# frank-xwang/InstanceDiffusion

Measured on AMD Instinct MI355X. Metric: images/sec at 512x512, 50 PLMS steps, N=8 instances (Multi-instance Sampler), higher is better.
Workload: dtype bf16; 1 GPU; C3: SD-1.5 InstanceDiffusion UNet (1.228B params, seeded random weights), 64x64 latent (512x512), 50 PLMS steps, CFG 7.5, N=8 boxes, MIS 0.36, alpha [0.8,0,0.2]; images_per_gpu=32, unet_forwards_per_image=406

## Files before the change

include/idf.h:

```cpp
#ifndef IDF_H_
#define IDF_H_

#include <stdint.h>

#ifdef __cplusplus
extern "C" {
#endif

#define IDF_ABI_VERSION 5

enum { IDF_BF16 = 0, IDF_F16 = 1 };
enum { IDF_E_ARG = -1, IDF_E_ALIGN = -2, IDF_E_UNSUPPORTED = -3 };

enum {
  IDF_EPI_BIAS     = 1,
  IDF_EPI_ROWBIAS  = 2,
  IDF_EPI_RES      = 4,
  IDF_EPI_GATE     = 8,
  IDF_EPI_SILU     = 16,
  IDF_EPI_GELU     = 32,
  IDF_EPI_GEGLU    = 64,
  IDF_EPI_OUT_F32  = 128,
  IDF_EPI_OUT_NCHW = 256,
  IDF_EPI_LN_ROW   = 512,
// ... 49 lines not shown

typedef struct {
  const void* x; const void* W; void* out;
  const float* bias; const void* rowbias; const void* res;
  int B, Hin, Win, Cin, Cout;
  int stride;
  int upsample;
  int ldx, ldo, ldr, ld_rowbias;
  int n_valid;
  int epi; int dtype;
  void* ws; long long ws_bytes;
  float* gn_partial;
} idf_conv3x3_args;
int idf_conv3x3(const idf_conv3x3_args* a, void* stream);
int idf_conv3x3_down(const idf_conv3x3_args* a, void* stream);

int idf_conv_in(const float* x_nchw, const float* w , const float* bias, void* out,
                int B, int Cin, int H, int W, int Cout, int dtype, void* stream);

typedef struct {
  const void* q; int ldq; long long strideQ; int nq;
  const void* k0; int ldk0; long long strideK0; const void* vt0; int ldv0; long long strideV0; int n0;
  const void* k1; int ldk1; long long strideK1; const void* vt1; int ldv1; long long strideV1; int n1;
  void* out; int ldo; long long strideO;
  int B, H, d;
  float scale;
  int dtype;
  const void* qbits; long long strideQb;
  const void* kbits0; long long strideKb0;
  const void* kbits1; long long strideKb1;
// ... 54 lines not shown
```

instancediffusion_amd/_lib.py:

```python
from __future__ import annotations

import ctypes as C
import os

_HERE = os.path.dirname(os.path.abspath(__file__))
LIB_PATH = os.environ.get("IDF_LIB_PATH", os.path.join(_HERE, "libidf_gfx950.so"))

IDF_BF16, IDF_F16 = 0, 1
IDF_STAT_GEMM_BIG_LAUNCHES, IDF_STAT_ATTN2_LAUNCHES, IDF_STAT_GEMM_RING_LAUNCHES, IDF_STAT_ATTN8_LAUNCHES, IDF_STAT_GN_EPI_LAUNCHES = 0, 1, 2, 3, 4
IDF_STAT_QKV_ROW_LAUNCHES, IDF_STAT_GEGLU_ROW_LAUNCHES = 6, 7
IDF_TUNE_GEMM_BIG, IDF_TUNE_ATTN2, IDF_TUNE_GEMM_RING, IDF_TUNE_BIG_MIN_EFF, IDF_TUNE_ATTN8, IDF_TUNE_MLP, IDF_TUNE_QKV_ROW, IDF_TUNE_GEGLU_ROW = 0, 1, 2, 3, 4, 5, 6, 7
EPI_LN_ROW, EPI_LN_COL, EPI_GEGLU_P32 = 512, 1024, 2048
EPI_BIAS, EPI_ROWBIAS, EPI_RES, EPI_GATE, EPI_SILU, EPI_GELU, EPI_GEGLU, EPI_OUT_F32, EPI_OUT_NCHW = \
    1, 2, 4, 8, 16, 32, 64, 128, 256

vp, ll, ci, cf = C.c_void_p, C.c_longlong, C.c_int, C.c_float


class GemmArgs(C.Structure):
    _fields_ = [("A", vp), ("W", vp), ("out", vp), ("bias", vp), ("rowbias", vp), ("res", vp), ("gate", vp),
                ("M", ci), ("N", ci), ("K", ci),
                ("lda", ci), ("ldw", ci), ("ldo", ci), ("ldr", ci), ("ld_rowbias", ci),
                ("rows_per_batch", ci),
                ("batch", ci), ("strideA", ll), ("strideW", ll), ("strideO", ll), ("strideR", ll),
                ("epi", ci), ("dtype", ci), ("ws", vp), ("ws_bytes", ll),
                ("ln_stats", vp), ("stride_ln_stats", ll), ("ln_c", vp), ("ln_d", vp),
                ("out_stats", vp), ("out_stats_eps", cf),
                ("ln_eps", cf), ("ln_stats_out", vp),
                ("vt_out", vp), ("ld_vt", ci), ("vt_col0", ci)]


class ConvArgs(C.Structure):
    _fields_ = [("x", vp), ("W", vp), ("out", vp), ("bias", vp), ("rowbias", vp), ("res", vp),
                ("B", ci), ("Hin", ci), ("Win", ci), ("Cin", ci), ("Cout", ci),
                ("stride", ci), ("upsample", ci),
                ("ldx", ci), ("ldo", ci), ("ldr", ci), ("ld_rowbias", ci),
                ("n_valid", ci), ("epi", ci), ("dtype", ci), ("ws", vp), ("ws_bytes", ll), ("gn_partial", vp)]


class AttnArgs(C.Structure):
    _fields_ = [("q", vp), ("ldq", ci), ("strideQ", ll), ("nq", ci),
                ("k0", vp), ("ldk0", ci), ("strideK0", ll), ("vt0", vp), ("ldv0", ci), ("strideV0", ll), ("n0", ci),
                ("k1", vp), ("ldk1", ci), ("strideK1", ll), ("vt1", vp), ("ldv1", ci), ("strideV1", ll), ("n1", ci),
                ("out", vp), ("ldo", ci), ("strideO", ll),
                ("B", ci), ("H", ci), ("d", ci), ("scale", cf), ("dtype", ci),
                ("qbits", vp), ("strideQb", ll), ("kbits0", vp), ("strideKb0", ll), ("kbits1", vp), ("strideKb1", ll)]


class MlpArgs(C.Structure):
    _fields_ = [("x", vp), ("ldx", ci), ("ln_stats", vp), ("w1", vp), ("ldw1", ci), ("cd", vp), ("w2p", vp), ("ldw2", ci),
                ("b2", vp), ("gate", vp), ("out", vp), ("ldo", ci), ("M", ci), ("C", ci), ("dtype", ci)]


SYMBOLS = {
    "idf_abi_version": (ci, []),
    "idf_build_info": (C.c_char_p, []),
    "idf_set_tuning": (ci, [ci, ci]),
    "idf_get_stat": (ll, [ci]),
    "idf_gemm": (ci, [C.POINTER(GemmArgs), vp]),
    "idf_conv3x3": (ci, [C.POINTER(ConvArgs), vp]),
    "idf_conv3x3_down": (ci, [C.POINTER(ConvArgs), vp]),
    "idf_mlp_geglu": (ci, [C.POINTER(MlpArgs), vp]),
    "idf_conv_in": (ci, [vp, vp, vp, vp, ci, ci, ci, ci, ci, ci, vp]),
    "idf_attention": (ci, [C.POINTER(AttnArgs), vp]),
    "idf_groupnorm_ws_floats": (ll, [ci, ci]),
    "idf_groupnorm": (ci, [vp, vp, vp, vp, vp, ci, ci, ci, cf, ci, ci, vp]),
    "idf_groupnorm_stats": (ci, [vp, vp, ci, ci, ci, ci, ci, vp]),
    "idf_groupnorm_apply": (ci, [vp, vp, vp, vp, vp, ci, ci, ci, ci, cf, ci, ci, vp]),
    "idf_layernorm": (ci, [vp, ci, vp, ci, vp, vp, ci, ci, cf, ci, vp]),
    "idf_row_stats": (ci, [vp, ci, vp, ci, ci, cf, ci, vp]),
    "idf_layernorm_patch2": (ci, [vp, vp, ci, vp, vp, ci, ci, ci, ci, cf, ci, vp]),
    "idf_seg_in_conv": (ci, [vp, vp, vp, vp, ci, ci, ci, ci, ci, vp]),
    "idf_dwconv7x7": (ci, [vp, vp, vp, vp, ci, ci, ci, ci, ci, vp]),
    "idf_scaleu_concat": (ci, [vp, vp, vp, vp, vp, vp, ci, ci, ci, ci, ci, ci, vp]),
    "idf_timestep_embedding": (ci, [vp, vp, ci, ci, ci, vp]),
    "idf_unifusion_embed": (ci, [vp, vp, vp, vp, vp, vp, vp, vp, ci, ci, ci, ci, vp]),
# ... 43 lines not shown
```

instancediffusion_amd/csrc/gemm_big.hip:

```cpp
#include "gemm_core.h"
#include <cstdlib>

using namespace idfcore;

namespace {

__device__ __attribute__((aligned(128))) unsigned short idf_zero_page[64];

#ifndef IDF_WAVE_ROWS
#define IDF_WAVE_ROWS 64
#endif
constexpr int WM = IDF_WAVE_ROWS, TM = WM / 32;
constexpr int NWAVES = 2 * 256 / WM;

template <int I> struct IC { static constexpr int value = I; };
template <int I, int N, int STEP, class F> __device__ __forceinline__ void static_for(F&& f) {
  if constexpr (I < N) { f(IC<I>{}); static_for<I + STEP, N, STEP>(f); }
}

typedef const __attribute__((address_space(1))) void* gptr_t;
typedef __attribute__((address_space(3))) void* lptr_t;

__device__ __forceinline__ unsigned lds_addr(const void* p) { return (unsigned)(size_t)p; }
__device__ __forceinline__ void dma16_sv(const void* sbase , unsigned voff_bytes, unsigned lds) {
// ... 425 lines not shown
#pragma unroll
          for (int j = 0; j < 4; ++j) {
            const f32x4 t = st4[j];
            v[2 * j] = t[1] * fmaf(-t[0], cn, v[2 * j]);
            v[2 * j + 1] = t[3] * fmaf(-t[2], cn, v[2 * j + 1]);
          }
        }
#pragma unroll
        for (int j = 0; j < 8; ++j) v[j] += bn;
        if (mb < p.M) *reinterpret_cast<u32x4*>(orow + mb) = pack8<DT>(v);
      }
    }
  });
}

#ifdef IDF_BIG_TRACE
__device__ unsigned long long idf_big_trace_buf[4][8];
#define TR_DECL unsigned long long tr_last = __builtin_readcyclecounter(), tr_acc[8] = {0, 0, 0, 0, 0, 0, 0, 0};
#define TR(i) { const unsigned long long tr_now = __builtin_readcyclecounter(); tr_acc[i] += tr_now - tr_last; tr_last = tr_now; }
#define TR_COUNT(i) { tr_acc[i] += 1; }
#define TR_DUMP { const int trb = blockIdx.x == 0 ? 0 : ((int)blockIdx.x == (int)gridDim.x / 2 ? 1 : -1);                     \
    if (trb >= 0 && lane == 0 && (wave == 0 || wave == NWAVES / 2)) { for (int i = 0; i < 8; ++i) idf_big_trace_buf[trb * 2 + (wave ? 1 : 0)][i] = tr_acc[i]; } }
#else
#define TR_DECL
#define TR(i)
#define TR_COUNT(i)
#define TR_DUMP
#endif

template <int DT, int BM, int BN, int BKT, int NSTG, bool CONV, bool SPLIT, bool LNS = false, bool VT = false, bool STATS = false,
          bool GLU = false, bool GST = false>
__global__ __launch_bounds__(64 * NWAVES, 1) void gemm_kernel_big(const CoreParams p, const int tiles_total) {
  constexpr int WN = BN / 2, TN = WN / 32;
  constexpr int NW = NWAVES;
  constexpr int RS = BKT;
  constexpr int CPR = BKT / 8;
  constexpr int RPI = 64 / CPR;
  constexpr int W_INST = BN / (RPI * NW), A_INST = BM / (RPI * NW);
  constexpr int DPW = W_INST + A_INST;
  constexpr int STAGE = (BM + BN) * RS;
  static_assert(BN % (RPI * NW) == 0 && BM % (RPI * NW) == 0, "tile rows must split evenly over the DMA instructions");
  extern __shared__ __attribute__((aligned(16))) unsigned short smem[];

  const int tid = threadIdx.x;
  const int lane = tid & 63, wave = __builtin_amdgcn_readfirstlane(tid >> 6);
  const int l31 = lane & 31, hi = lane >> 5;
// ... 13 lines not shown
  const int full = SPLIT ? p.full_items : tiles_total;
  auto item_map = [&](int item, int& tile, int& slice, int& nki) {
    if (!SPLIT || item < full) { tile = item; slice = 0; nki = SPLIT ? p.kt_full : nk; }
    else { const int r = item - full; const int t = r / S; tile = full + t; slice = r - t * S; nki = nk; }
  };

  const int dr = lane / CPR, dc = lane % CPR;
  auto swz = [](int row) { return CPR == 8 ? ((row >> 1) & 7) : ((row >> 2) & 3); };
  unsigned woff[W_INST], aoff[A_INST];
  int ayx[A_INST];
  int l_seq, l_kt = 0, l_k0 = 0, l_nk = 0, tap = 0, ci0 = 0;

  auto setup_loader = [&](int item) {
    int tile, slice;
    item_map(item, tile, slice, l_nk);
    const int m_tile = tile / tiles_n;
    const int n0 = (tile - m_tile * tiles_n) * BN, m0 = m_tile * BM;
    l_k0 = slice * nk;
#pragma unroll
    for (int j = 0; j < W_INST; ++j) {
      const int row = RPI * (wave + NW * j) + dr;
      woff[j] = (unsigned)(n0 + row) * (unsigned)p.ldw + (unsigned)((dc ^ swz(row)) * 8);
    }
#pragma unroll
    for (int j = 0; j < A_INST; ++j) {
      const int row = RPI * (wave + NW * j) + dr;
      const int m = min(m0 + row, p.M - 1);
      const unsigned sw = (unsigned)((dc ^ swz(row)) * 8);
      if (CONV) {
        const int hw = p.Ho * p.Wo;
        const int b = m / hw, rem = m - b * hw;
        const int yo = rem / p.Wo, xo = rem - yo * p.Wo;
        const int y0 = yo * p.stride - p.pad_lo, x0 = xo * p.stride - p.pad_lo;
        if (p.up == 0) {
          int mask = 0;
#pragma unroll
          for (int t = 0; t < 9; ++t) {
            const int yi = y0 + t / 3, xi = x0 + t % 3;
            mask |= ((yi >= 0) & (yi < p.Hin) & (xi >= 0) & (xi < p.Win)) << t;
          }
          ayx[j] = mask;
          aoff[j] = (unsigned)b * (unsigned)(p.Hin * p.Win) * (unsigned)p.lda + (unsigned)((y0 * p.Win + x0) * p.lda) + sw;
        } else {
          ayx[j] = (y0 << 16) | (x0 & 0xffff);
          aoff[j] = (unsigned)b * (unsigned)(p.Hin * p.Win) * (unsigned)p.lda + sw;
        }
      } else {
// ... 1 lines not shown
        aoff[j] = (unsigned)m * (unsigned)p.lda + sw;
      }
    }
    if (CONV) { const int k_elem = l_k0 * BKT; tap = k_elem / p.Cin; ci0 = k_elem - tap * p.Cin; }
  };

  auto issue_piece = [&](int stage, auto II) {
    constexpr int i = decltype(II)::value;
    unsigned short* Al = smem + stage * STAGE;
    if constexpr (i < W_INST) {
      constexpr int j = i;
      dma16_sv(p.W + (size_t)(l_k0 + l_kt) * BKT, woff[j] * 2u, lds_addr(Al + BM * RS + RPI * (wave + NW * j) * RS));
    } else {
      constexpr int j = i - W_INST;
      const unsigned dst = lds_addr(Al + RPI * (wave + NW * j) * RS);
      if (CONV && p.up == 0) {
        const int ky = tap / 3, kx = tap - ky * 3;
        const unsigned tapoff = (unsigned)((ky * p.Win + kx) * p.lda + ci0);
        const bool ok = (ayx[j] >> tap) & 1;
        const unsigned short* src = ok ? p.A + (aoff[j] + tapoff) : idf_zero_page + dc * 8;
        dma16_v(src, dst);
      } else if (CONV) {
        const int ky = tap / 3, kx = tap - ky * 3;
        const int Hup = p.Hin << p.up, Wup = p.Win << p.up;
        const int yi = (ayx[j] >> 16) + ky, xi = (int)(short)(ayx[j] & 0xffff) + kx;
        const bool ok = (yi >= 0) & (yi < Hup) & (xi >= 0) & (xi < Wup);
        const int ys = yi >> p.up, xs = xi >> p.up;
        const unsigned short* src = ok ? p.A + ci0 + (aoff[j] + (unsigned)(ys * p.Win + xs) * (unsigned)p.lda) : idf_zero_page + dc * 8;
        dma16_v(src, dst);
      } else {
        dma16_sv(p.A + (size_t)(l_k0 + l_kt) * BKT, aoff[j] * 2u, dst);
// ... 103 lines not shown
#pragma unroll
  for (int j = 0; j < NSTG - 1; ++j)
    if (l_seq < seq_end) { issue_dma(j); ++issued; }
  int it = 0, st_it = 0;
  int young_stores = 0;
  TR_DECL
  const int epi = p.epi;
  const float gate = (epi & IDF_EPI_GATE) ? p.gate[0] : 0.0f;
  char* const stg = reinterpret_cast<char*>(smem + NSTG * STAGE) + wave * 2048;

  auto run_tile = [&](auto SWAPT, auto SPLT) {
    constexpr bool SWAP = decltype(SWAPT)::value;
    constexpr bool SPL = decltype(SPLT)::value;
    int tile, slice, nki;
    item_map(seq, tile, slice, nki);
    f32x16 acc[TN][TM];
    float lsx[TM], lsq[TM];
#pragma unroll
    for (int a = 0; a < TN; ++a)
#pragma unroll
      for (int b = 0; b < TM; ++b)
#pragma unroll
        for (int r = 0; r < 16; ++r) acc[a][b][r] = 0.0f;
#pragma unroll
    for (int b = 0; b < TM; ++b) { lsx[b] = 0.0f; lsq[b] = 0.0f; }
    TR(5) TR_COUNT(7)

    for (int kt = 0; kt < nki; ++kt) {
      if (NSTG > 2 && issued - it == NSTG - 1) asm volatile("s_waitcnt vmcnt(%0)" ::"n"((NSTG - 2) * DPW) : "memory");
      else if (NSTG == 2 && kt == 0 && young_stores > 0) {
// ... 37 lines not shown
      }
    }
    if constexpr (SWAP) {
      if constexpr (LNS) {
        float* stw = reinterpret_cast<float*>(stg);
        if (hi == 0) {
#pragma unroll
          for (int b = 0; b < TM; ++b) *reinterpret_cast<f32x2*>(stw + 2 * (b * 32 + l31)) = f32x2{lnm[b], lnr[b]};
        }
        asm volatile("s_waitcnt lgkmcnt(0)" ::: "memory");
        __builtin_amdgcn_wave_barrier();
        big_epilogue_vt<DT, BM, BN, TN>(p, acc, seq, tiles_n, wm, wn, l31, hi, stw, (seq / tiles_n) * BM + wm * WM);
      } else {
        big_epilogue_vt<DT, BM, BN, TN>(p, acc, seq, tiles_n, wm, wn, l31, hi, p.ln_stats, 0);
      }
    } else {
      big_epilogue<DT, BM, BN, TN, SPL, LNS, STATS, GLU, GST>(p, acc, tile, slice, tiles_n, wm, wn, l31, hi, gate, stg, lnm, lnr);
    }
    TR(4)
    young_stores = 0;
    if (p.epi_vmcnt && (tile / tiles_n) * BM + BM <= p.M) {
      if constexpr (SWAP) young_stores = 2 * TN * TM;
      else if constexpr (SPL) young_stores = 4 * TN * TM;
      else if constexpr (GLU) young_stores = TN * TM;
      else young_stores = (epi & IDF_EPI_GEGLU) ? TN * TM : ((epi & IDF_EPI_OUT_F32) ? 4 * TN * TM : 2 * TN * TM);
    }
  };

  for (; seq < seq_end; seq += seq_step) {
    if constexpr (VT) {
// ... 29 lines not shown
      const int v = atoi(e);
      return (v < lo || v > hi) ? dflt : v;
    };
    BigSched c;
    c.walk = env("IDF_BIG_WALK", 2, 0, 2);
    c.dephase = env("IDF_BIG_DEPHASE", 0, 0, 16);
    c.dephase_min_rounds = env("IDF_BIG_DEPHASE_MIN_ROUNDS", 8, 1, 1 << 20);
    c.dephase_epi_cycles = env("IDF_BIG_DEPHASE_EPI", 6000, 0, 1 << 20);
    c.epi_vmcnt = env("IDF_BIG_EPIVM", 1, 0, 1);
    return c;
  }();
  return sc;
}

template <int DT, int BN, int NSTG, bool CONV, bool SPLIT = false, bool LNS = false, bool VT = false, bool STATS = false, bool GLU = false,
          bool GST = false>
int launch_big_cfg(const CoreParams& p, hipStream_t s, int splitk = 1) {
  constexpr int BM = 256, BKT = 64;
  if constexpr (!SPLIT && !LNS && !VT && !STATS && !GLU && !GST && NSTG == 2) {
    if (splitk > 1) return launch_big_cfg<DT, BN, NSTG, CONV, true>(p, s, splitk);
  }
  if constexpr (!SPLIT && !LNS && !CONV && !STATS && !GST && NSTG == 2) {
    if ((p.epi & IDF_EPI_LN_ROW) && !p.ln_stats) return launch_big_cfg<DT, BN, NSTG, CONV, false, true, VT, false, GLU>(p, s, 1);
  }
  void (*kern)(const CoreParams, const int) = gemm_kernel_big<DT, BM, BN, BKT, NSTG, CONV, SPLIT, LNS, VT, STATS, GLU, GST>;
  constexpr int smem = NSTG * (BM + BN) * BKT * 2 + NWAVES * 2048;
  static std::atomic<unsigned long long> attr_done{0};
  if (const int e = idf_lds_optin(reinterpret_cast<const void*>(kern), smem, attr_done)) return e;
  CoreParams q = p;
  q.splitk = splitk; q.kt_per_slice = p.K / BKT / splitk; q.kt_full = p.K / BKT;
  const int tiles_all = (p.N / BN) * ((p.M + BM - 1) / BM);
  if (!SPLIT) { q.full_items = tiles_all; q.tail_m0 = 0; q.tail_rows = p.M; }
  const int tiles = q.full_items + (tiles_all - q.full_items) * splitk;
  const int slots = num_cu();
  const int grid = tiles < slots ? tiles : slots;
  {
    const BigSched& sc = big_sched();
    const int rounds = (tiles + slots - 1) / slots;
    q.tile_walk = (!SPLIT && (sc.walk == 1 || (sc.walk == 2 && p.N / BN >= 32))) ? 1 : 0;
    q.epi_vmcnt = sc.epi_vmcnt;
    q.dephase = 0; q.dephase_units = 0;
    if (!SPLIT && sc.dephase > 1 && rounds >= sc.dephase_min_rounds) {
      q.dephase = sc.dephase;
      q.dephase_units = (q.kt_full * 3400 + sc.dephase_epi_cycles) / 1024;
    }
  }
  hipLaunchKernelGGL(kern, dim3(grid), dim3(64 * NWAVES), smem, s, q, tiles);
  return idf_launch_status();
// ... 107 lines not shown
  if (stats) return bn == 320 ? launch_big_cfg<DT, 320, 2, false, false, false, false, true>(ps, s)                        \
                              : launch_big_cfg<DT, 256, 2, false, false, false, false, true>(ps, s);                       \
  if (vt) return launch_big_cfg<DT, 320, 2, false, false, false, true>(p, s);                                             \
  if (bn == 128) {                         \
    if (conv) return launch_big_cfg<DT, 128, 3, true>(p, s);                                                              \
    return launch_big_cfg<DT, 128, 3, false>(p, s);                                                                       \
  }                                                                                                                       \
  if (gst) return launch_big_cfg<DT, 320, 2, true, false, false, false, false, false, true>(p, s);                         \
  if (conv) return bn == 320 ? launch_big_cfg<DT, 320, 2, true>(pq, s, splitk) : launch_big_cfg<DT, 256, 2, true>(pq, s, splitk);   \
  return bn == 320 ? launch_big_cfg<DT, 320, 2, false>(pq, s, splitk) : launch_big_cfg<DT, 256, 2, false>(pq, s, splitk);
  if (dtype == IDF_BF16) { IDF_BIG_DISPATCH(IDF_BF16) }
  if (dtype == IDF_F16) { IDF_BIG_DISPATCH(IDF_F16) }
#undef IDF_BIG_DISPATCH
  return IDF_E_UNSUPPORTED;
}
```

instancediffusion_amd/csrc/gemm_conv.hip:

```cpp
#include "gemm_core.h"
#include "attn_core.h"
#include <cstdlib>

using namespace idfcore;

namespace {

#ifndef IDF_GEMM_BIG_DEFAULT
#define IDF_GEMM_BIG_DEFAULT 1
#endif
constexpr int LSTR = 72;

template <int DT, int BM, int BN, int WM, int WN, int KLOOP_LDS_BYTES>
__device__ __forceinline__ void tile_epilogue(const CoreParams& p, f32x16 (&acc)[WN / 32][WM / 32], unsigned short* smem,
                                              int m0, int n0, int bz, int wm, int wn, int lane, int wave) {
  constexpr int TM = WM / 32, TN = WN / 32;
  const int l31 = lane & 31, hi = lane >> 5;
  constexpr int CSTR = WN + 4;
  static_assert(4 * WM * CSTR * 4 <= KLOOP_LDS_BYTES, "C staging must fit in the allocated LDS");
  __syncthreads();
  float* Cl = reinterpret_cast<float*>(smem) + wave * (WM * CSTR);
#pragma unroll
  for (int a = 0; a < TN; ++a)
#pragma unroll
// ... 975 lines not shown
  int gst = 0, rc = IDF_E_UNSUPPORTED;
  if (a->dtype == IDF_BF16) rc = launch<IDF_BF16, true>(p, 1, s, nullptr, &gst);
  else if (a->dtype == IDF_F16) rc = launch<IDF_F16, true>(p, 1, s, nullptr, &gst);
  if (rc == 0 && gst) ++idf_stat_gn_epi_launches;
  if (rc == 0 && a->gn_partial && !gst)
    rc = idf_groupnorm_stats(a->out, a->gn_partial, a->B, p.Ho * p.Wo, a->Cout, p.Ho * p.Wo / 64, a->dtype, stream);
  return rc;
}

extern "C" int idf_conv3x3(const idf_conv3x3_args* a, void* stream) { return conv3x3_launch(a, 1, stream); }

extern "C" int idf_conv3x3_down(const idf_conv3x3_args* a, void* stream) {
  if (!a || a->stride != 2 || a->upsample != 0 || a->Hin < 2 || a->Win < 2) return IDF_E_ARG;
  return conv3x3_launch(a, 0, stream);
}
```

instancediffusion_amd/csrc/gemm_core.h:

```cpp
#pragma once
#include "common.h"
#include <atomic>

namespace idfcore {

struct CoreParams {
  const unsigned short* W; int ldw; long long strideW; int N;
  const unsigned short* A; int lda; long long strideA; int M; int K;
  int Hin, Win, Cin, Ho, Wo, stride, up;
  void* out; int ldo; long long strideO;
  const float* bias; const unsigned short* rowbias; int ld_rowbias; int rows_per_batch;
  const unsigned short* res; int ldr; long long strideR;
  const float* gate; int epi; int n_valid;
  float* ws; size_t ws_bytes; int splitk; int kt_per_slice;
  int full_items; int kt_full; int tail_m0; int tail_rows;
  const float* ln_stats; long long stride_ln_stats; const float* ln_c; const float* ln_d;
  float ln_eps; float* ln_stats_out;
  unsigned short* vt_out; int ld_vt; int vt_col0;
  float* stat_parts; int parts;
  float* gn_partial; int gn_hw;
  int tile_walk; int dephase; int dephase_units; int epi_vmcnt;
  int pad_lo;
};

constexpr int BK = 64;

template <int DT>
__device__ __forceinline__ void epilogue8(const CoreParams& p, int bz, int m, int n, float* v, float gate) {
  const int epi = p.epi;
  const bool full = (n + 7 < p.N);
  if (epi & IDF_EPI_LN_ROW) {
    const f32x2 st = *reinterpret_cast<const f32x2*>(p.ln_stats + (size_t)bz * p.stride_ln_stats + 2 * (size_t)m);
#pragma unroll
    for (int e = 0; e < 8; ++e) if (n + e < p.N) v[e] = st[1] * fmaf(-st[0], p.ln_c[n + e], v[e]);
  }
  if (epi & IDF_EPI_LN_COL) {
    const float cm = p.ln_c[m], dm = p.ln_d[m];
// ... 66 lines not shown
      *reinterpret_cast<u32x4*>(o) = pack8<DT>(v);
    } else {
#pragma unroll
      for (int e = 0; e < 8; ++e) if (n + e < p.N) o[e] = Elem<DT>::from_f32(v[e]);
    }
  }
}


}

#define IDF_BIG_UNSUPPORTED (-100)
extern std::atomic<long long> idf_stat_big_launches;
int idf_launch_big(const idfcore::CoreParams& p, int dtype, bool conv, bool force, hipStream_t s, int* splitk_out,
                   int* parts_out = nullptr, int* tail_m0_out = nullptr, int* gst_out = nullptr);
int idf_launch_qkv320w(const idfcore::CoreParams& p, int dtype, hipStream_t s);
int idf_launch_geglu640w(const idfcore::CoreParams& p, int dtype, hipStream_t s);
int idf_gegluw_set_mode(int v);
int idf_launch_qkv640w(const idfcore::CoreParams& p, int dtype, hipStream_t s);
int idf_qkvw_set_mode(int v);
int idf_mlp_set_mode(int v);
int idf_big_min_eff_pct(int set);
int idf_num_cu();
int idf_stats_finalize(const float* stat_parts, int parts, int cols_per_part, float* out_stats, int M, float eps, hipStream_t s);
```

instancediffusion_amd/engine.py:

```python
from __future__ import annotations

import os
from typing import Dict, List, Optional, Sequence, Tuple

import torch

from .host.attention import SpatialTransformer
from .host.unet import Downsample, ResBlock, UNetModel, Upsample

LN_SELF_MODE = int(os.environ.get("IDF_LN_SELF", "1"))
if LN_SELF_MODE not in (0, 1, 2):
    raise ValueError(f"IDF_LN_SELF={LN_SELF_MODE}: must be 0, 1 or 2")
QKV_ROW = os.environ.get("IDF_QKV_ROW", "1") != "0"
OBJ_TOKENS = 184
MASK_RES = 64


def _round_up(x: int, m: int) -> int:
    return (x + m - 1) // m * m


GEGLU_PERIOD = int(os.environ.get("IDF_GEGLU_PERIOD", "32"))
if GEGLU_PERIOD not in (32, 64):
    raise ValueError(f"IDF_GEGLU_PERIOD={GEGLU_PERIOD}: must be 32 or 64")
MLP_FUSED = os.environ.get("IDF_MLP_FUSED", "1")
if MLP_FUSED not in ("0", "1"):
    raise ValueError(f"IDF_MLP_FUSED={MLP_FUSED}: must be 0 or 1")
MLP_FUSED = MLP_FUSED == "1" and GEGLU_PERIOD == 32
MLP_MIN_M = int(os.environ.get("IDF_MLP_MIN_M", "32768"))
PAIR_HOIST = os.environ.get("IDF_PAIR_HOIST", "1")
if PAIR_HOIST not in ("0", "1"):
    raise ValueError(f"IDF_PAIR_HOIST={PAIR_HOIST}: must be 0 or 1")
PAIR_HOIST = PAIR_HOIST == "1"
GN_EPI = os.environ.get("IDF_GN_EPI", "1")
if GN_EPI not in ("0", "1"):
    raise ValueError(f"IDF_GN_EPI={GN_EPI}: must be 0 or 1")
GN_EPI = GN_EPI == "1"
DEBUG_PAIRED = os.environ.get("IDF_DEBUG_PAIRED", "0") == "1"


def pack_geglu(w: torch.Tensor, b: torch.Tensor, period: int = 64) -> Tuple[torch.Tensor, torch.Tensor]:
    n2, k = w.shape
    n = n2 // 2
    h = period // 2
    assert n % h == 0
    wv, wg = w[:n].reshape(n // h, h, k), w[n:].reshape(n // h, h, k)
    bv, bg = b[:n].reshape(n // h, h), b[n:].reshape(n // h, h)
    return torch.cat([wv, wg], dim=1).reshape(n2, k).contiguous(), torch.cat([bv, bg], dim=1).reshape(n2).contiguous()


def pack_conv3x3(w: torch.Tensor) -> torch.Tensor:
    co, ci = w.shape[0], w.shape[1]
    return w.permute(0, 2, 3, 1).reshape(co, 9 * ci).contiguous()


class _Lin:
    __slots__ = ("w", "b")

    def __init__(self, w, b):
        self.w, self.b = w, b


class Cond:

    _next_uid = 0

    def __init__(self, B: int):
        Cond._next_uid += 1
# ... 75 lines not shown
    def _w16(self, t: torch.Tensor) -> torch.Tensor:
        return t.detach().to(device=self.device, dtype=torch.float32).to(self.dtype).contiguous()

    def _f32(self, t: torch.Tensor) -> torch.Tensor:
        return t.detach().to(device=self.device, dtype=torch.float32).contiguous()

    def _lin(self, m, with_bias=True) -> _Lin:
        w = m.weight
        if w.dim() == 4:
            w = w.reshape(w.shape[0], w.shape[1])
        return _Lin(self._w16(w), self._f32(m.bias) if (with_bias and m.bias is not None) else None)

    def _conv(self, m) -> _Lin:
        return _Lin(self._w16(pack_conv3x3(m.weight.detach().float())), self._f32(m.bias))

    def _fold_ln(self, w: torch.Tensor, bias, norm):
        w = w.detach().float()
        g, b = norm.weight.detach().float(), norm.bias.detach().float()
        w16 = self._w16(w * g[None, :])
        d = w @ b + (bias.detach().float() if bias is not None else 0.0)
        return w16, w16.float().sum(1).contiguous(), self._f32(d)

    def _pack_ff(self, ff, norm):
        w = ff.net[0].proj.weight.detach().float()
        g, b = norm.weight.detach().float(), norm.bias.detach().float()
        wp, dp = pack_geglu(w * g[None, :], ff.net[0].proj.bias.detach().float() + w @ b, GEGLU_PERIOD)
        w16 = self._w16(wp)
        f = dict(w1=w16, b1=self._f32(dp), c1=w16.float().sum(1).contiguous(), l2=self._lin(ff.net[2]))
        C = w.shape[1]
        if MLP_FUSED and hasattr(self.ops, "mlp_geglu") and self.ops.mlp_supported(128, C):
# ... 47 lines not shown
                    f_lin=self._lin(fz.linear), f_attn=self._attn(fz.attn, fz.norm1, True), f_kv=self._attn_kv_plain(fz.attn),
                    f_ff=self._pack_ff(fz.ff, fz.norm2),
                    f_n1=(self._f32(fz.norm1.weight), self._f32(fz.norm1.bias)),
                    f_n2=(self._f32(fz.norm2.weight), self._f32(fz.norm2.bias)))

    def _pack_layers(self, seq, emb_w, emb_b, off, tanh_alphas):
        out = []
        for _, layer in seq.items():
            if isinstance(layer, ResBlock):
                out.append(self._pack_res(layer, emb_w, emb_b, off))
            elif isinstance(layer, SpatialTransformer):
                out.append(self._pack_st(layer, tanh_alphas))
            elif isinstance(layer, Downsample):
                out.append(dict(kind="down", conv=self._conv(layer.op)))
            elif isinstance(layer, Upsample):
                out.append(dict(kind="up", conv=self._conv(layer.conv)))
            else:
                out.append(dict(kind="conv_in", w=self._f32(layer.weight), b=self._f32(layer.bias)))
        return out

    def _pack(self, model: UNetModel):
        emb_w, emb_b, off, tanh_alphas = [], [], [0], []
        self.te0 = self._lin(model.time_embed[0])
        self.te2 = self._lin(model.time_embed[2])
        self.in_blocks = [self._pack_layers(b, emb_w, emb_b, off, tanh_alphas) for b in model.input_blocks]
        self.mid_block = self._pack_layers(model.middle_block, emb_w, emb_b, off, tanh_alphas)
        self.out_blocks = [self._pack_layers(b, emb_w, emb_b, off, tanh_alphas) for b in model.output_blocks]
        self.emb_all = _Lin(self._w16(torch.cat(emb_w, 0)), self._f32(torch.cat(emb_b, 0)))
        self.emb_total = off[0]
        self.tanh_alphas = torch.stack(tanh_alphas).to(self.device)
        self.gates = torch.zeros_like(self.tanh_alphas)
# ... 345 lines not shown
                B, _, H, W = x_nchw.shape
                h = self.ops.conv_in(x_nchw, p["w"], p["b"], self.buf(out_role, (B, H, W, p["w"].shape[0])))
                gnp = None
            elif k == "res":
                h, gnp = self._res(p, h, emb_all, out_role, gnp, want_out=norm_next)
            elif k == "st":
                h = self._st(p, h, cond, fuser_on, dup=dup_st, gnp=gnp)
                gnp = None
            elif k == "down":
                B, H, W, C = h.shape
                Ho, Wo = (H + 1) // 2, (W + 1) // 2
                gnp = self._gnp("gnp.out", B, Ho * Wo, C) if norm_next else None
                h = self.ops.conv3x3(h, p["conv"].w, self.buf(out_role, (B, Ho, Wo, C)), bias=p["conv"].b, stride=2, gn_partial=gnp)
            elif k == "up":
                B, H, W, C = h.shape
                h = self.ops.conv3x3(h, p["conv"].w, self.buf(out_role + ".up", (B, 2 * H, 2 * W, C)),
                                     bias=p["conv"].b, upsample=1)
                gnp = None
        return h, gnp

    def _forward_ops(self, x: torch.Tensor, t_f32: torch.Tensor, cond: Cond, eps: torch.Tensor, fuser_on: bool,
                     paired: bool = False):
        ops = self.ops
        B = x.shape[0]
        hoist = (paired and PAIR_HOIST and B % 2 == 0 and len(self.in_blocks) > 1
                 and [p["kind"] for p in self.in_blocks[0]] == ["conv_in"] and [p["kind"] for p in self.in_blocks[1]] == ["res", "st"])
        n = B // 2
        mc = self.model.model_channels
        te = ops.timestep_embedding(t_f32, self.buf("temb.sin", (B, mc)))
        e1 = ops.gemm(te, self.te0.w, self.buf("temb.1", (B, 4 * mc)), bias=self.te0.b, act="silu")
        es = ops.gemm(e1, self.te2.w, self.buf("temb.2", (B, 4 * mc)), bias=self.te2.b, act="silu")
        emb_all = ops.gemm(es, self.emb_all.w, self.buf("temb.all", (B, self.emb_total)), bias=self.emb_all.b)
# ... 110 lines not shown
```

instancediffusion_amd/ops.py:

```python
from __future__ import annotations

import ctypes as C
from typing import Optional

import torch

from . import _lib
from ._lib import (EPI_BIAS, EPI_GATE, EPI_GEGLU, EPI_GEGLU_P32, EPI_GELU, EPI_LN_COL, EPI_LN_ROW, EPI_OUT_F32, EPI_OUT_NCHW,
                   EPI_RES, EPI_ROWBIAS, EPI_SILU)

_DT = {torch.bfloat16: _lib.IDF_BF16, torch.float16: _lib.IDF_F16}


def _p(t: Optional[torch.Tensor]):
    return None if t is None else C.c_void_p(t.data_ptr())


def _rows2d(t: torch.Tensor):
    assert t.stride(-1) == 1 or t.shape[-1] == 1, "last dim must be contiguous"
    return t.stride(-2), (t.stride(0) if t.dim() == 3 else 0)


class HipOps:

# ... 186 lines not shown
        args = _lib.ConvArgs(
            x=x.data_ptr(), W=w.data_ptr(), out=out.data_ptr(),
            bias=None if bias is None else bias.data_ptr(), rowbias=None,
            res=None if res is None else res.data_ptr(),
            B=B, Hin=H, Win=W_, Cin=Cin, Cout=Cout, stride=2, upsample=0,
            ldx=x.stride(2), ldo=out.stride(2), ldr=0 if res is None else res.stride(2),
            ld_rowbias=0, n_valid=0, epi=epi, dtype=self.dt,
            ws=self._splitk_ws().data_ptr(), ws_bytes=self.SPLITK_WS_BYTES,
            gn_partial=None if gn_partial is None else gn_partial.data_ptr())
        if gn_partial is not None:
            assert gn_partial.dtype == torch.float32 and gn_partial.is_contiguous() and out.is_contiguous()
            assert tuple(gn_partial.shape) == self.gn_partial_shape(out.shape[0], out.shape[1] * out.shape[2], Cout)
        _lib.check(self.lib.idf_conv3x3_down(C.byref(args), self._stream()), "idf_conv3x3_down")
        return out

    def conv_in(self, x_nchw, w, bias, out):
        B, Cin, H, W_ = x_nchw.shape
        assert x_nchw.dtype == torch.float32 and x_nchw.is_contiguous() and out.is_contiguous()
        _lib.check(self.lib.idf_conv_in(_p(x_nchw), _p(w), _p(bias), _p(out), B, Cin, H, W_, out.shape[-1], self.dt,
                                        self._stream()), "idf_conv_in")
        return out

    def attention(self, q, k0, vt0, n0, out, heads, *, k1=None, vt1=None, n1=0, qbits=None, kbits0=None, kbits1=None):
        if qbits is not None:
            for t in (qbits, kbits0) + ((kbits1,) if n1 else ()):
                assert t.dtype == torch.int32 and t.stride(-1) == 1 and t.dim() == 2
        B, Nq, Cc = q.shape
        d = Cc // heads
        a = _lib.AttnArgs(
            q=q.data_ptr(), ldq=q.stride(1), strideQ=q.stride(0), nq=Nq,
# ... 149 lines not shown
```

Baseline: 2.126 img/s.

## Fold nearest-upsample into 3x3 conv as four 2x2 phase convolutions

Adds a folded upsample path. A nearest 2x upsample followed by a 3x3 conv is rewritten as four sub-pixel phase convolutions, each with a 2x2 kernel over the low-resolution input, using weights pre-summed on the host. The big GEMM kernel gains a FOLD mode that maps tiles to phases, loads only the 4 taps of the low-res input, and scatters results to the interleaved high-res output rows. This cuts the conv's reduction length from 9*Cin to 4*Cin and avoids reading the upsampled input, at the cost of a new kernel variant. It falls back to the old conv when the shape is unsupported, for example when N is not a multiple of 320 or grid efficiency is too low.

```diff
diff --git a/include/idf.h b/include/idf.h
--- a/include/idf.h
+++ b/include/idf.h
@@ -87,6 +87,7 @@
 } idf_conv3x3_args;
 int idf_conv3x3(const idf_conv3x3_args* a, void* stream);
 int idf_conv3x3_down(const idf_conv3x3_args* a, void* stream);
+int idf_conv_up2x_folded(const idf_conv3x3_args* a, void* stream);
 
 int idf_conv_in(const float* x_nchw, const float* w , const float* bias, void* out,
                 int B, int Cin, int H, int W, int Cout, int dtype, void* stream);
diff --git a/instancediffusion_amd/_lib.py b/instancediffusion_amd/_lib.py
--- a/instancediffusion_amd/_lib.py
+++ b/instancediffusion_amd/_lib.py
@@ -30,6 +30,9 @@
                 ("vt_out", vp), ("ld_vt", ci), ("vt_col0", ci)]
 
 
+E_UNSUPPORTED = -3
+
+
 class ConvArgs(C.Structure):
     _fields_ = [("x", vp), ("W", vp), ("out", vp), ("bias", vp), ("rowbias", vp), ("res", vp),
                 ("B", ci), ("Hin", ci), ("Win", ci), ("Cin", ci), ("Cout", ci),
@@ -60,6 +63,7 @@
     "idf_gemm": (ci, [C.POINTER(GemmArgs), vp]),
     "idf_conv3x3": (ci, [C.POINTER(ConvArgs), vp]),
     "idf_conv3x3_down": (ci, [C.POINTER(ConvArgs), vp]),
+    "idf_conv_up2x_folded": (ci, [C.POINTER(ConvArgs), vp]),
     "idf_mlp_geglu": (ci, [C.POINTER(MlpArgs), vp]),
     "idf_conv_in": (ci, [vp, vp, vp, vp, ci, ci, ci, ci, ci, ci, vp]),
     "idf_attention": (ci, [C.POINTER(AttnArgs), vp]),
diff --git a/instancediffusion_amd/csrc/gemm_big.hip b/instancediffusion_amd/csrc/gemm_big.hip
--- a/instancediffusion_amd/csrc/gemm_big.hip
+++ b/instancediffusion_amd/csrc/gemm_big.hip
@@ -463,6 +463,53 @@
   });
 }
 
+template <int DT, int BM, int BN, int TN>
+__device__ __forceinline__ void big_epilogue_fold(const CoreParams& p, f32x16 (&acc)[TN][TM], int tile, int ph, int tiles_n, int wm,
+                                                  int wn, int l31_in, int hi_in) {
+  constexpr int WN = BN / 2;
+  int l31 = l31_in, hi = hi_in;
+  asm volatile("" : "+v"(l31), "+v"(hi));
+  const int m_tile = tile / tiles_n;
+  const int n0 = (tile - m_tile * tiles_n) * BN, m0 = m_tile * BM;
+  const int mw = m0 + wm * WM, nw = n0 + wn * WN;
+  const int ph_row = (ph >> 1) * 2 * p.Wo + (ph & 1);
+  unsigned short* orow[TM];
+#pragma unroll
+  for (int b = 0; b < TM; ++b) {
+    const int m = min(mw + b * 32 + l31, p.M - 1);
+    const int x = m % p.Wo;
+    orow[b] = reinterpret_cast<unsigned short*>(p.out) + (size_t)(4 * m - 2 * x + ph_row) * p.ldo;
+  }
+  static_for<0, TN, 1>([&](auto AI) {
+    constexpr int a = decltype(AI)::value;
+    const int n = nw + a * 32 + 16 * hi;
+    f32x4 bs[4];
+    if (p.epi & IDF_EPI_BIAS) {
+#pragma unroll
+      for (int j = 0; j < 4; ++j) bs[j] = *reinterpret_cast<const f32x4*>(p.bias + n + 4 * j);
+    }
+#pragma unroll
+    for (int b = 0; b < TM; ++b) {
+      float v[16];
+#pragma unroll
+      for (int e = 0; e < 4; ++e) {
+        const auto s02 = __builtin_amdgcn_permlane32_swap(__float_as_uint(acc[a][b][e]), __float_as_uint(acc[a][b][8 + e]), false, false);
+        const auto s13 = __builtin_amdgcn_permlane32_swap(__float_as_uint(acc[a][b][4 + e]), __float_as_uint(acc[a][b][12 + e]), false, false);
+        v[e] = __uint_as_float(s02[0]); v[4 + e] = __uint_as_float(s02[1]);
+        v[8 + e] = __uint_as_float(s13[0]); v[12 + e] = __uint_as_float(s13[1]);
+      }
+      if (p.epi & IDF_EPI_BIAS) {
+#pragma unroll
+        for (int j = 0; j < 16; ++j) v[j] += bs[j >> 2][j & 3];
+      }
+      if (mw + b * 32 + l31 < p.M) {
+        *reinterpret_cast<u32x4*>(orow[b] + n) = pack8<DT>(v);
+        *reinterpret_cast<u32x4*>(orow[b] + n + 8) = pack8<DT>(v + 8);
+      }
+    }
+  });
+}
+
 #ifdef IDF_BIG_TRACE
 __device__ unsigned long long idf_big_trace_buf[4][8];
 #define TR_DECL unsigned long long tr_last = __builtin_readcyclecounter(), tr_acc[8] = {0, 0, 0, 0, 0, 0, 0, 0};
@@ -478,7 +525,7 @@
 #endif
 
 template <int DT, int BM, int BN, int BKT, int NSTG, bool CONV, bool SPLIT, bool LNS = false, bool VT = false, bool STATS = false,
-          bool GLU = false, bool GST = false>
+          bool GLU = false, bool GST = false, bool FOLD = false>
 __global__ __launch_bounds__(64 * NWAVES, 1) void gemm_kernel_big(const CoreParams p, const int tiles_total) {
   constexpr int WN = BN / 2, TN = WN / 32;
   constexpr int NW = NWAVES;
@@ -522,13 +569,16 @@
   auto setup_loader = [&](int item) {
     int tile, slice;
     item_map(item, tile, slice, l_nk);
+    [[maybe_unused]] int ph = 0;
+    if constexpr (FOLD) { ph = tile / p.fold_tiles; tile -= ph * p.fold_tiles; }
     const int m_tile = tile / tiles_n;
     const int n0 = (tile - m_tile * tiles_n) * BN, m0 = m_tile * BM;
     l_k0 = slice * nk;
 #pragma unroll
     for (int j = 0; j < W_INST; ++j) {
       const int row = RPI * (wave + NW * j) + dr;
-      woff[j] = (unsigned)(n0 + row) * (unsigned)p.ldw + (unsigned)((dc ^ swz(row)) * 8);
+      if constexpr (FOLD) woff[j] = (unsigned)(ph * p.N + n0 + row) * (unsigned)p.ldw + (unsigned)((dc ^ swz(row)) * 8);
+      else woff[j] = (unsigned)(n0 + row) * (unsigned)p.ldw + (unsigned)((dc ^ swz(row)) * 8);
     }
 #pragma unroll
     for (int j = 0; j < A_INST; ++j) {
@@ -539,6 +589,18 @@
         const int hw = p.Ho * p.Wo;
         const int b = m / hw, rem = m - b * hw;
         const int yo = rem / p.Wo, xo = rem - yo * p.Wo;
+        if constexpr (FOLD) {
+          const int y0 = yo - 1 + (ph >> 1), x0 = xo - 1 + (ph & 1);
+          int mask = 0;
+#pragma unroll
+          for (int t = 0; t < 4; ++t) {
+            const int yi = y0 + (t >> 1), xi = x0 + (t & 1);
+            mask |= ((yi >= 0) & (yi < p.Hin) & (xi >= 0) & (xi < p.Win)) << t;
+          }
+          ayx[j] = mask;
+          aoff[j] = (unsigned)b * (unsigned)(p.Hin * p.Win) * (unsigned)p.lda + (unsigned)((y0 * p.Win + x0) * p.lda) + sw;
+          continue;
+        }
         const int y0 = yo * p.stride - p.pad_lo, x0 = xo * p.stride - p.pad_lo;
         if (p.up == 0) {
           int mask = 0;
@@ -570,7 +632,12 @@
     } else {
       constexpr int j = i - W_INST;
       const unsigned dst = lds_addr(Al + RPI * (wave + NW * j) * RS);
-      if (CONV && p.up == 0) {
+      if constexpr (FOLD) {
+        const unsigned tapoff = (unsigned)(((tap >> 1) * p.Win + (tap & 1)) * p.lda + ci0);
+        const bool ok = (ayx[j] >> tap) & 1;
+        const unsigned short* src = ok ? p.A + (aoff[j] + tapoff) : idf_zero_page + dc * 8;
+        dma16_v(src, dst);
+      } else if (CONV && p.up == 0) {
         const int ky = tap / 3, kx = tap - ky * 3;
         const unsigned tapoff = (unsigned)((ky * p.Win + kx) * p.lda + ci0);
         const bool ok = (ayx[j] >> tap) & 1;
@@ -704,6 +771,8 @@
     constexpr bool SPL = decltype(SPLT)::value;
     int tile, slice, nki;
     item_map(seq, tile, slice, nki);
+    [[maybe_unused]] int ph = 0;
+    if constexpr (FOLD) { ph = tile / p.fold_tiles; tile -= ph * p.fold_tiles; }
     f32x16 acc[TN][TM];
     float lsx[TM], lsq[TM];
 #pragma unroll
@@ -771,6 +840,8 @@
       } else {
         big_epilogue_vt<DT, BM, BN, TN>(p, acc, seq, tiles_n, wm, wn, l31, hi, p.ln_stats, 0);
       }
+    } else if constexpr (FOLD) {
+      big_epilogue_fold<DT, BM, BN, TN>(p, acc, tile, ph, tiles_n, wm, wn, l31, hi);
     } else {
       big_epilogue<DT, BM, BN, TN, SPL, LNS, STATS, GLU, GST>(p, acc, tile, slice, tiles_n, wm, wn, l31, hi, gate, stg, lnm, lnr);
     }
@@ -830,16 +901,16 @@
 }
 
 template <int DT, int BN, int NSTG, bool CONV, bool SPLIT = false, bool LNS = false, bool VT = false, bool STATS = false, bool GLU = false,
-          bool GST = false>
+          bool GST = false, bool FOLD = false>
 int launch_big_cfg(const CoreParams& p, hipStream_t s, int splitk = 1) {
   constexpr int BM = 256, BKT = 64;
-  if constexpr (!SPLIT && !LNS && !VT && !STATS && !GLU && !GST && NSTG == 2) {
+  if constexpr (!SPLIT && !LNS && !VT && !STATS && !GLU && !GST && !FOLD && NSTG == 2) {
     if (splitk > 1) return launch_big_cfg<DT, BN, NSTG, CONV, true>(p, s, splitk);
   }
   if constexpr (!SPLIT && !LNS && !CONV && !STATS && !GST && NSTG == 2) {
     if ((p.epi & IDF_EPI_LN_ROW) && !p.ln_stats) return launch_big_cfg<DT, BN, NSTG, CONV, false, true, VT, false, GLU>(p, s, 1);
   }
-  void (*kern)(const CoreParams, const int) = gemm_kernel_big<DT, BM, BN, BKT, NSTG, CONV, SPLIT, LNS, VT, STATS, GLU, GST>;
+  void (*kern)(const CoreParams, const int) = gemm_kernel_big<DT, BM, BN, BKT, NSTG, CONV, SPLIT, LNS, VT, STATS, GLU, GST, FOLD>;
   constexpr int smem = NSTG * (BM + BN) * BKT * 2 + NWAVES * 2048;
   static std::atomic<unsigned long long> attr_done{0};
   if (const int e = idf_lds_optin(reinterpret_cast<const void*>(kern), smem, attr_done)) return e;
@@ -847,7 +918,8 @@
   q.splitk = splitk; q.kt_per_slice = p.K / BKT / splitk; q.kt_full = p.K / BKT;
   const int tiles_all = (p.N / BN) * ((p.M + BM - 1) / BM);
   if (!SPLIT) { q.full_items = tiles_all; q.tail_m0 = 0; q.tail_rows = p.M; }
-  const int tiles = q.full_items + (tiles_all - q.full_items) * splitk;
+  int tiles = q.full_items + (tiles_all - q.full_items) * splitk;
+  if constexpr (FOLD) { q.fold_tiles = tiles_all; tiles = 4 * tiles_all; }
   const int slots = num_cu();
   const int grid = tiles < slots ? tiles : slots;
   {
@@ -985,3 +1057,23 @@
 #undef IDF_BIG_DISPATCH
   return IDF_E_UNSUPPORTED;
 }
+
+int idf_launch_big_fold(const CoreParams& p, int dtype, bool force, hipStream_t s) {
+  if (p.Cin <= 0 || (p.Cin % BK) != 0 || p.K != 4 * p.Cin || p.ldw != p.K) return IDF_BIG_UNSUPPORTED;
+  if ((p.N % 320) != 0 || p.n_valid != p.N || (p.epi & ~IDF_EPI_BIAS)) return IDF_BIG_UNSUPPORTED;
+  if ((p.lda % 8) || (p.ldo % 8) || !aligned16(p.A) || !aligned16(p.W) || !aligned16(p.out)) return IDF_BIG_UNSUPPORTED;
+  if ((p.epi & IDF_EPI_BIAS) && !aligned16(p.bias)) return IDF_BIG_UNSUPPORTED;
+  if (p.Ho != p.Hin || p.Wo != p.Win || p.M <= 0 || (p.M % (p.Hin * p.Win)) != 0) return IDF_BIG_UNSUPPORTED;
+  const long long slots = (long long)num_cu();
+  const long long items = 4ll * (p.N / 320) * ((p.M + 255) / 256);
+  if (!force) {
+    const long long rounds = (items + slots - 1) / slots;
+    if ((double)items / (double)(rounds * slots) * 100.0 < (double)idf_big_min_eff_pct(-1)) return IDF_BIG_UNSUPPORTED;
+  }
+  if ((unsigned long long)p.M * (unsigned long long)p.lda >= (1ull << 31) || 4ull * p.N * p.ldw >= (1ull << 31) ||
+      items >= (1ll << 30) || (unsigned long long)p.M * 4ull >= (1ull << 31)) return IDF_BIG_UNSUPPORTED;
+  ++idf_stat_big_launches;
+  if (dtype == IDF_BF16) return launch_big_cfg<IDF_BF16, 320, 2, true, false, false, false, false, false, false, true>(p, s);
+  if (dtype == IDF_F16) return launch_big_cfg<IDF_F16, 320, 2, true, false, false, false, false, false, false, true>(p, s);
+  return IDF_E_UNSUPPORTED;
+}
diff --git a/instancediffusion_amd/csrc/gemm_conv.hip b/instancediffusion_amd/csrc/gemm_conv.hip
--- a/instancediffusion_amd/csrc/gemm_conv.hip
+++ b/instancediffusion_amd/csrc/gemm_conv.hip
@@ -1013,3 +1013,23 @@
   if (!a || a->stride != 2 || a->upsample != 0 || a->Hin < 2 || a->Win < 2) return IDF_E_ARG;
   return conv3x3_launch(a, 0, stream);
 }
+
+extern "C" int idf_conv_up2x_folded(const idf_conv3x3_args* a, void* stream) {
+  if (!a || !a->x || !a->W || !a->out) return IDF_E_ARG;
+  if (a->B <= 0 || a->Hin <= 0 || a->Win <= 0 || a->Cin <= 0 || (a->Cin % BK) != 0 || a->Cout <= 0) return IDF_E_ARG;
+  if (a->stride != 1 || a->upsample != 1) return IDF_E_ARG;
+  if ((a->epi & ~IDF_EPI_BIAS) || a->rowbias || a->res || a->gn_partial || a->n_valid) return IDF_E_ARG;
+  if ((a->epi & IDF_EPI_BIAS) && !a->bias) return IDF_E_ARG;
+  if ((a->ldx % 8) || (a->ldo % 8) || !aligned16(a->x) || !aligned16(a->W) || !aligned16(a->out)) return IDF_E_ALIGN;
+  if (a->dtype != IDF_BF16 && a->dtype != IDF_F16) return IDF_E_UNSUPPORTED;
+  const int big = gemm_big_mode();
+  if (big == 0) return IDF_E_UNSUPPORTED;
+  CoreParams p{};
+  p.W = (const unsigned short*)a->W; p.ldw = 4 * a->Cin; p.N = a->Cout; p.n_valid = a->Cout;
+  p.A = (const unsigned short*)a->x; p.lda = a->ldx; p.K = 4 * a->Cin;
+  p.Hin = a->Hin; p.Win = a->Win; p.Cin = a->Cin; p.Ho = a->Hin; p.Wo = a->Win; p.stride = 1; p.up = 0; p.pad_lo = 1;
+  p.M = a->B * a->Hin * a->Win;
+  p.out = a->out; p.ldo = a->ldo; p.bias = a->bias; p.epi = a->epi; p.rows_per_batch = a->Hin * a->Win;
+  const int rc = idf_launch_big_fold(p, a->dtype, big == 2, (hipStream_t)stream);
+  return rc == IDF_BIG_UNSUPPORTED ? IDF_E_UNSUPPORTED : rc;
+}
diff --git a/instancediffusion_amd/csrc/gemm_core.h b/instancediffusion_amd/csrc/gemm_core.h
--- a/instancediffusion_amd/csrc/gemm_core.h
+++ b/instancediffusion_amd/csrc/gemm_core.h
@@ -21,6 +21,7 @@
   float* gn_partial; int gn_hw;
   int tile_walk; int dephase; int dephase_units; int epi_vmcnt;
   int pad_lo;
+  int fold_tiles;
 };
 
 constexpr int BK = 64;
@@ -117,6 +118,7 @@
 extern std::atomic<long long> idf_stat_big_launches;
 int idf_launch_big(const idfcore::CoreParams& p, int dtype, bool conv, bool force, hipStream_t s, int* splitk_out,
                    int* parts_out = nullptr, int* tail_m0_out = nullptr, int* gst_out = nullptr);
+int idf_launch_big_fold(const idfcore::CoreParams& p, int dtype, bool force, hipStream_t s);
 int idf_launch_qkv320w(const idfcore::CoreParams& p, int dtype, hipStream_t s);
 int idf_launch_geglu640w(const idfcore::CoreParams& p, int dtype, hipStream_t s);
 int idf_gegluw_set_mode(int v);
diff --git a/instancediffusion_amd/engine.py b/instancediffusion_amd/engine.py
--- a/instancediffusion_amd/engine.py
+++ b/instancediffusion_amd/engine.py
@@ -36,6 +36,10 @@
 if GN_EPI not in ("0", "1"):
     raise ValueError(f"IDF_GN_EPI={GN_EPI}: must be 0 or 1")
 GN_EPI = GN_EPI == "1"
+UP_FOLD = os.environ.get("IDF_UP_FOLD", "1")
+if UP_FOLD not in ("0", "1"):
+    raise ValueError(f"IDF_UP_FOLD={UP_FOLD}: must be 0 or 1")
+UP_FOLD = UP_FOLD == "1"
 DEBUG_PAIRED = os.environ.get("IDF_DEBUG_PAIRED", "0") == "1"
 
 
@@ -52,6 +56,22 @@
 def pack_conv3x3(w: torch.Tensor) -> torch.Tensor:
     co, ci = w.shape[0], w.shape[1]
     return w.permute(0, 2, 3, 1).reshape(co, 9 * ci).contiguous()
+
+
+def pack_conv_up2x(w: torch.Tensor) -> torch.Tensor:
+    assert w.dim() == 4 and tuple(w.shape[2:]) == (3, 3) and w.dtype == torch.float32
+    co, ci = w.shape[0], w.shape[1]
+    rows = ((w[:, :, 0], w[:, :, 1] + w[:, :, 2]), (w[:, :, 0] + w[:, :, 1], w[:, :, 2]))
+    out = w.new_empty(4, co, 4 * ci)
+    for py in range(2):
+        for px in range(2):
+            taps = []
+            for ty in range(2):
+                r = rows[py][ty]
+                cols = (r[:, :, 0], r[:, :, 1] + r[:, :, 2]) if px == 0 else (r[:, :, 0] + r[:, :, 1], r[:, :, 2])
+                taps += [cols[0], cols[1]]
+            out[py * 2 + px] = torch.stack(taps, dim=1).reshape(co, 4 * ci)
+    return out
 
 
 class _Lin:
@@ -157,6 +177,16 @@
     def _conv(self, m) -> _Lin:
         return _Lin(self._w16(pack_conv3x3(m.weight.detach().float())), self._f32(m.bias))
 
+    def _pack_up(self, m) -> dict:
+        if UP_FOLD and hasattr(self.ops, "conv_up2x"):
+            return dict(kind="up", conv=None, fold=self._w16(pack_conv_up2x(m.weight.detach().float())), b=self._f32(m.bias), mod=m)
+        return dict(kind="up", conv=self._conv(m), fold=None)
+
+    def _up_conv3(self, p) -> _Lin:
+        if p["conv"] is None:
+            p["conv"] = self._conv(p["mod"])
+        return p["conv"]
+
     def _fold_ln(self, w: torch.Tensor, bias, norm):
         w = w.detach().float()
         g, b = norm.weight.detach().float(), norm.bias.detach().float()
@@ -234,7 +264,7 @@
             elif isinstance(layer, Downsample):
                 out.append(dict(kind="down", conv=self._conv(layer.op)))
             elif isinstance(layer, Upsample):
-                out.append(dict(kind="up", conv=self._conv(layer.conv)))
+                out.append(self._pack_up(layer.conv))
             else:
                 out.append(dict(kind="conv_in", w=self._f32(layer.weight), b=self._f32(layer.bias)))
         return out
@@ -610,8 +640,11 @@
                 h = self.ops.conv3x3(h, p["conv"].w, self.buf(out_role, (B, Ho, Wo, C)), bias=p["conv"].b, stride=2, gn_partial=gnp)
             elif k == "up":
                 B, H, W, C = h.shape
-                h = self.ops.conv3x3(h, p["conv"].w, self.buf(out_role + ".up", (B, 2 * H, 2 * W, C)),
-                                     bias=p["conv"].b, upsample=1)
+                up = self.buf(out_role + ".up", (B, 2 * H, 2 * W, C))
+                if p["fold"] is None or not self.ops.conv_up2x(h, p["fold"], up, bias=p["b"]):
+                    conv = self._up_conv3(p)
+                    self.ops.conv3x3(h, conv.w, up, bias=conv.b, upsample=1)
+                h = up
                 gnp = None
         return h, gnp
 
diff --git a/instancediffusion_amd/ops.py b/instancediffusion_amd/ops.py
--- a/instancediffusion_amd/ops.py
+++ b/instancediffusion_amd/ops.py
@@ -224,6 +224,24 @@
         _lib.check(self.lib.idf_conv3x3_down(C.byref(args), self._stream()), "idf_conv3x3_down")
         return out
 
+    def conv_up2x(self, x, wf, out, *, bias=None) -> bool:
+        B, H, W_, Cin = x.shape
+        assert x.stride(-1) == 1 and x.stride(1) == W_ * x.stride(2) and x.stride(0) == H * x.stride(1)
+        Cout = wf.shape[1]
+        assert tuple(wf.shape) == (4, Cout, 4 * Cin) and wf.is_contiguous() and wf.dtype == self.dtype
+        assert tuple(out.shape) == (B, 2 * H, 2 * W_, Cout) and out.stride(-1) == 1 and out.dtype == self.dtype
+        assert out.stride(1) == out.shape[2] * out.stride(2) and out.stride(0) == out.shape[1] * out.stride(1)
+        args = _lib.ConvArgs(
+            x=x.data_ptr(), W=wf.data_ptr(), out=out.data_ptr(), bias=None if bias is None else bias.data_ptr(),
+            rowbias=None, res=None, B=B, Hin=H, Win=W_, Cin=Cin, Cout=Cout, stride=1, upsample=1,
+            ldx=x.stride(2), ldo=out.stride(2), ldr=0, ld_rowbias=0, n_valid=0, epi=0 if bias is None else EPI_BIAS,
+            dtype=self.dt, ws=None, ws_bytes=0, gn_partial=None)
+        rc = self.lib.idf_conv_up2x_folded(C.byref(args), self._stream())
+        if rc == _lib.E_UNSUPPORTED:
+            return False
+        _lib.check(rc, "idf_conv_up2x_folded")
+        return True
+
     def conv_in(self, x_nchw, w, bias, out):
         B, Cin, H, W_ = x_nchw.shape
         assert x_nchw.dtype == torch.float32 and x_nchw.is_contiguous() and out.is_contiguous()
```

After: 2.181 img/s, median of 6. 2.6% higher.
